# NVlabs/UMR

Hardware: NVIDIA H100
Metric: render fwd+bwd images/sec @256x256 1280-face mesh (higher is better)
Workload: dtype f32

## Files before the change

umr_b200/csrc/raster.cu:

```cuda
#include <cuda_runtime.h>
#include <stdint.h>

#include "common.cuh"
#include "umr_b200.h"

namespace umr {

constexpr int TILE = 16;
constexpr int CTA = TILE * TILE;
constexpr int CHUNK = 32;
constexpr int NSTAGE = 2;
constexpr int REC_F = 32;

constexpr int R_V = 0;
constexpr int R_INV = 9;
constexpr int R_SYM = 18;
constexpr int R_BOX = 24;
constexpr int R_FLG = 28;
constexpr int R_IZ2 = 29;

constexpr int NARROW_MAX_FACES = 65535;
template <typename IdxT>
__host__ __device__ constexpr int hdr_shift() { return sizeof(IdxT) == 2 ? 16 : 24; }
constexpr int FACE_WINDOW = 65536;
// ... 89 lines not shown
    if (valid) {
        float4* dst = reinterpret_cast<float4*>(rec + (size_t)i * REC_F);
#pragma unroll
        for (int k = 0; k < REC_F / 4; ++k)
            dst[k] = make_float4(out[4 * k], out[4 * k + 1], out[4 * k + 2], out[4 * k + 3]);
        box[i] = make_float4(xlo, xhi, ylo, yhi);
    }
    uint32_t k0 = ubox_key(xhi), k1 = ubox_key(-xlo), k2 = ubox_key(yhi), k3 = ubox_key(-ylo);
#pragma unroll
    for (int o = 16; o > 0; o >>= 1) {
        k0 = max(k0, __shfl_xor_sync(0xffffffffu, k0, o));
        k1 = max(k1, __shfl_xor_sync(0xffffffffu, k1, o));
        k2 = max(k2, __shfl_xor_sync(0xffffffffu, k2, o));
        k3 = max(k3, __shfl_xor_sync(0xffffffffu, k3, o));
    }
    if ((threadIdx.x & 31) == 0) {
        uint32_t* u = ubox + (size_t)blockIdx.y * 4;
        atomicMax(u + 0, k0); atomicMax(u + 1, k1); atomicMax(u + 2, k2); atomicMax(u + 3, k3);
    }
}

__device__ __forceinline__ bool tile_outside_union(const uint32_t* __restrict__ ubox, int b, const float* s_ext) {
    const uint4 u = __ldg(reinterpret_cast<const uint4*>(ubox) + b);
    if (u.x == 0xffffffffu || u.y == 0xffffffffu || u.z == 0xffffffffu || u.w == 0xffffffffu) return false;
    const float xhi = __uint_as_float(u.x), xlo = -__uint_as_float(u.y);
    const float yhi = __uint_as_float(u.z), ylo = -__uint_as_float(u.w);
    return s_ext[0] > xhi || s_ext[1] < xlo || s_ext[2] > yhi || s_ext[3] < ylo;
}

struct Frag {
    float w0, w1, w2;
    float t0, t1, t2;
    float sign, dx, dy, dis, D;
};

__device__ __forceinline__ float pixel_coord(int i, int S) {
    return __fdiv_rn((float)(2 * i + 1 - S), (float)S);
}

__device__ __forceinline__ bool fragment(const float* __restrict__ rc, float xp, float yp, float thr,
                                         float sigma, Frag& fr) {
    const float w0 = rc[R_INV + 0] * xp + rc[R_INV + 1] * yp + rc[R_INV + 2];
    const float w1 = rc[R_INV + 3] * xp + rc[R_INV + 4] * yp + rc[R_INV + 5];
    const float w2 = rc[R_INV + 6] * xp + rc[R_INV + 7] * yp + rc[R_INV + 8];
    fr.w0 = w0; fr.w1 = w1; fr.w2 = w2;
    const float fx0 = rc[0], fy0 = rc[1], fx1 = rc[3], fy1 = rc[4], fx2 = rc[6], fy2 = rc[7];
    const float s00 = rc[R_SYM + 0], s01 = rc[R_SYM + 1], s02 = rc[R_SYM + 2];
    const float s11 = rc[R_SYM + 3], s12 = rc[R_SYM + 4], s22 = rc[R_SYM + 5];
    float dx, dy, t0, t1, t2;
    if (w0 > 0 && w1 > 0 && w2 > 0 && w0 < 1 && w1 < 1 && w2 < 1) {
        float best = 100000000.f;
        {
            const float a0 = s00 - s01, a1 = s01 - s11, a2 = s02 - s12;
            float u0 = (w0 * a0 + w1 * a1 + w2 * a2 - a1) / (a0 - a1);
            float u1 = 1 - u0;
            float u2 = 0;
            u0 -= w0; u1 -= w1; u2 -= w2;
            const float ex = u0 * fx0 + u1 * fx1 + u2 * fx2;
            const float ey = u0 * fy0 + u1 * fy1 + u2 * fy2;
            const float d = ex * ex + ey * ey;
            dx = 0.f; dy = 0.f; t0 = t1 = t2 = 0.f;
            if (d < best) { best = d; dx = ex; dy = ey; t0 = u0; t1 = u1; t2 = u2; }
        }
        {
            const float a0 = s01 - s02, a1 = s11 - s12, a2 = s12 - s22;
            float u1 = (w0 * a0 + w1 * a1 + w2 * a2 - a2) / (a1 - a2);
            float u2 = 1 - u1;
            float u0 = 0;
            u0 -= w0; u1 -= w1; u2 -= w2;
            const float ex = u0 * fx0 + u1 * fx1 + u2 * fx2;
            const float ey = u0 * fy0 + u1 * fy1 + u2 * fy2;
            const float d = ex * ex + ey * ey;
            if (d < best) { best = d; dx = ex; dy = ey; t0 = u0; t1 = u1; t2 = u2; }
        }
        {
            const float a0 = s02 - s00, a1 = s12 - s01, a2 = s22 - s02;
            float u2 = (w0 * a0 + w1 * a1 + w2 * a2 - a0) / (a2 - a0);
            float u0 = 1 - u2;
            float u1 = 0;
            u0 -= w0; u1 -= w1; u2 -= w2;
            const float ex = u0 * fx0 + u1 * fx1 + u2 * fx2;
            const float ey = u0 * fy0 + u1 * fy1 + u2 * fy2;
            const float d = ex * ex + ey * ey;
            if (d < best) { best = d; dx = ex; dy = ey; t0 = u0; t1 = u1; t2 = u2; }
        }
        fr.sign = 1.f;
    } else {
        const uint32_t flg = __float_as_uint(rc[R_FLG]);
        int v0 = -1;
        if (w1 <= 0 && w2 <= 0) {
            v0 = 0;
            if ((flg & 1u) && (xp - fx0) * (fx2 - fx0) + (yp - fy0) * (fy2 - fy0) > 0) v0 = 2;
        } else if (w2 <= 0 && w0 <= 0) {
            v0 = 1;
            if ((flg & 2u) && (xp - fx1) * (fx0 - fx1) + (yp - fy1) * (fy0 - fy1) > 0) v0 = 0;
        } else if (w0 <= 0 && w1 <= 0) {
            v0 = 2;
            if ((flg & 4u) && (xp - fx2) * (fx1 - fx2) + (yp - fy2) * (fy1 - fy2) > 0) v0 = 1;
        } else if (w0 <= 0) v0 = 1;
        else if (w1 <= 0) v0 = 2;
        else if (w2 <= 0) v0 = 0;
        if (v0 < 0) v0 = w0 >= w1 ? (w0 >= w2 ? 0 : 2) : (w1 >= w2 ? 1 : 2);
        float u0, u1, u2;
        if (v0 == 0) {
            const float a0 = s00 - s01, a1 = s01 - s11, a2 = s02 - s12;
            u0 = (w0 * a0 + w1 * a1 + w2 * a2 - a1) / (a0 - a1);
            u1 = 1 - u0;
            u2 = 0;
        } else if (v0 == 1) {
            const float a0 = s01 - s02, a1 = s11 - s12, a2 = s12 - s22;
            u1 = (w0 * a0 + w1 * a1 + w2 * a2 - a2) / (a1 - a2);
            u2 = 1 - u1;
            u0 = 0;
        } else {
            const float a0 = s02 - s00, a1 = s12 - s01, a2 = s22 - s02;
            u2 = (w0 * a0 + w1 * a1 + w2 * a2 - a0) / (a2 - a0);
            u0 = 1 - u2;
            u1 = 0;
        }
        u0 = fminf(fmaxf(u0, 0.f), 1.f) - w0;
        u1 = fminf(fmaxf(u1, 0.f), 1.f) - w1;
        u2 = fminf(fmaxf(u2, 0.f), 1.f) - w2;
        t0 = u0; t1 = u1; t2 = u2;
        dx = t0 * fx0 + t1 * fx1 + t2 * fx2;
        dy = t0 * fy0 + t1 * fy1 + t2 * fy2;
        fr.sign = -1.f;
    }
    const float dis = dx * dx + dy * dy;
    if (fr.sign < 0 && dis >= thr) return false;
    fr.t0 = t0; fr.t1 = t1; fr.t2 = t2;
    fr.dx = dx; fr.dy = dy; fr.dis = dis;
    const float e = expf(-fr.sign * dis / sigma);
    fr.D = (float)(1. / (1. + (double)e));
    return true;
}


__device__ __forceinline__ void clip_bary(float& w0, float& w1, float& w2) {
    const float hi = (float)(1 - 1e-5), lo = (float)1e-5;
    w0 = fmaxf(fminf(w0, hi), lo);
    w1 = fmaxf(fminf(w1, hi), lo);
    w2 = fmaxf(fminf(w2, hi), lo);
    const float s = fmaxf(w0 + w1 + w2, lo);
    w0 /= s; w1 /= s; w2 /= s;
}

__device__ __forceinline__ float depth_of(const float* __restrict__ rc, float c0, float c1, float c2) {
    return __fdiv_rn(1.f, c0 / rc[2] + c1 / rc[5] + c2 / rc[8]);
}

__device__ __forceinline__ int texel_index(float c0, float c1, int R) {
    const int wx = (int)(c0 * R);
    const int wy = (int)(c1 * R);
    if ((c0 + c1) * R - wx - wy <= 1) return wy * R + wx;
    return (R - 1 - wy) * R + (R - 1 - wx);
}

struct Consts {
    float thr, sigma, gamma, near_, far_, inv_unused;
    float r_sigma, r_gamma, r_fn, r_nf;
    int F, T2, R, S, IS, aa, double_side;
    int dist, alpha, tex;
    int vec_store;
    size_t tex_bs;
    int tex_div;
};

constexpr int P2F_LIMBS = 4;
constexpr int P2F_LIMB_BITS = 26;
constexpr int P2F_FRAC_BITS = 96;
constexpr int P2F_DET_WORDS = 3 * P2F_LIMBS + 1;

__device__ __forceinline__ void red_add_u64(unsigned long long* addr, unsigned long long v) {
    asm volatile("red.global.add.u64 [%0], %1;" ::"l"(addr), "l"(v) : "memory");
}

__device__ __forceinline__ void red_fixed(unsigned long long* limbs, unsigned long long* bad, float v) {
// ... 1228 lines not shown
                        const float* aggrs_info, const float* grad_images, float* grad_faces, float* grad_textures,
                        const Consts& K, const PairBuf& pb) {
#define UMR_BWD2_GO(GEOMV, PREV) \
    k_raster_bwd2<RGBM, TG, TS, 3, GEOMV, PREV, IdxT><<<grid, BWD2_THREADS, 0, stream>>>(rec, textures, soft_colors, aggrs_info, grad_images, \
                                                                                    grad_faces, grad_textures, K, pb)
    if constexpr (TG && RGBM == 1) {
        if (pre) { if (grad_faces) UMR_BWD2_GO(true, true); else UMR_BWD2_GO(false, true); }
        else { if (grad_faces) UMR_BWD2_GO(true, false); else UMR_BWD2_GO(false, false); }
    } else if constexpr (TG) {
        if (grad_faces) UMR_BWD2_GO(true, false); else UMR_BWD2_GO(false, false);
    } else {
        UMR_BWD2_GO(true, false);
    }
#undef UMR_BWD2_GO
}

static int forward_impl(int tile_mode) { return tile_mode == 32 ? 4 : 3; }

extern "C" size_t umr_raster_workspace_bytes(int32_t B, int32_t F, int32_t image_size, int32_t anti_aliasing) {
    if (B <= 0 || F <= 0 || image_size <= 0) return 0;
    return ws_layout(B, F, image_size * (anti_aliasing ? 2 : 1)).total;
}

constexpr size_t PAIR_BLOCK_RESERVE = 1540;
extern "C" size_t umr_raster_pair_buffer_bytes(int32_t B, int32_t image_size, int32_t anti_aliasing,
                                               uint64_t capacity_blocks) {
    if (B <= 0 || image_size <= 0) return 0;
    const size_t blk = (size_t)BLK_F4 * sizeof(float4) + sizeof(uint32_t);
    return pair_layout(B, image_size * (anti_aliasing ? 2 : 1), (size_t)capacity_blocks).total +
           (size_t)capacity_blocks * (PAIR_BLOCK_RESERVE - blk) + 1024;
}

static int pair_texel_bits(const UmrRasterParams* p) {
    return (p->color_channels != 4 && forward_impl(p->tile_mode) == 4) ? 21 : 23;
}

static PairBuf make_pairbuf(const UmrRasterParams* p, int S) {
    PairBuf pb;
    pb.ctrl = nullptr; pb.tile_head = nullptr; pb.ulist = nullptr; pb.blk_hdr = nullptr; pb.recs = nullptr; pb.cap = 0;
    if (!p->pair_buffer || p->pair_buffer_bytes == 0 || ((uintptr_t)p->pair_buffer & 255) != 0) return pb;
    if (p->texture_size > (1 << pair_texel_bits(p))) return pb;
    size_t cap = pair_capacity(p->batch_size, S, (size_t)p->pair_buffer_bytes);
    if (cap > 0x7fff0000u) cap = 0x7fff0000u;
    if (cap < 4) return pb;
    const PairBufLayout L = pair_layout(p->batch_size, S, cap);
    char* base = (char*)p->pair_buffer;
    pb.ctrl = (uint32_t*)(base + L.ctrl_off);
    pb.tile_head = (int32_t*)(base + L.head_off);
    pb.ulist = (int32_t*)(base + L.ulist_off);
    pb.blk_hdr = (uint32_t*)(base + L.hdr_off);
    pb.recs = (float4*)(base + L.rec_off);
    pb.cap = (uint32_t)cap;
    return pb;
}

constexpr double TEXGRAD_PRE_RATIO_FULL = 160.0, TEXGRAD_PRE_RATIO_TEXONLY = 120.0;
static bool is_generic(const UmrRasterParams* p);
static int check_params(const UmrRasterParams* p) {
    if (!p) return UMR_ERR_BAD_ARG;
    if (p->batch_size <= 0 || p->num_faces <= 0 || p->texture_size <= 0 || p->image_size <= 0)
        return UMR_ERR_BAD_ARG;
    if (p->num_faces > UMR_RASTER_MAX_FACES || p->batch_size > 65535) return UMR_ERR_TOO_LARGE;
    if (p->func_id_dist < 0 || p->func_id_dist > 2 || p->func_id_alpha < 0 || p->func_id_alpha > 2 ||
        p->texture_sample_type < 0 || p->texture_sample_type > 1)
        return UMR_ERR_UNSUPPORTED;
    if (p->texture_sample_type == UMR_TEX_VERTEX && p->texture_size != 3) return UMR_ERR_BAD_ARG;
    if (p->shared_textures > 1 && p->batch_size % p->shared_textures != 0) return UMR_ERR_BAD_ARG;
// ... 441 lines not shown
```

umr_b200/csrc/raster_fwd3.cuh:

```cuda
#pragma once

namespace umr {

constexpr int FWD3_CTAS = 4;

template <int RGB, int NC = 3, typename IdxT = uint16_t, bool DET = false>
__global__ void __launch_bounds__(CTA, FWD3_CTAS) k_raster_fwd3(const float* __restrict__ rec_all, const float4* __restrict__ box_all,
                                                        const IdxT* __restrict__ clist, const int* __restrict__ ccount,
                                                        const float* __restrict__ textures, float* __restrict__ images,
                                                        float* __restrict__ colors_hi, float* __restrict__ aggrs,
                                                        float* __restrict__ p2f_acc, const uint32_t* __restrict__ ubox,
                                                        Consts K, float eps, float bg0, float bg1, float bg2, PairBuf pb,
                                                        int ncb, float bg3 = 0.f,
                                                        uint8_t* __restrict__ vis_mask = nullptr) {
    constexpr int NPL = NC + 1;
    constexpr bool VIS = RGB == 2;
    const float bgc[4] = {bg0, bg1, bg2, bg3};
    constexpr int WG = 16;
    __shared__ __align__(128) float s_wrec[NWARP * 2 * WG * REC_F];
    float* s_rec = s_wrec;
    __shared__ IdxT s_list[LCAP];
    __shared__ uint8_t s_meet[LCAP];
    __shared__ uint32_t s_boff[LCAP + 1];
    __shared__ float s_xp[TILE], s_yp[TILE], s_ext[4];
// ... 262 lines not shown
            for (int r = 0; mm; ++r) {
                const int e = __ffs(mm) - 1;
                mm &= mm - 1u;
                const int jl = base + e;
                const uint32_t meet = s_meet[jl];
                const float* rc = stage + r * REC_F;
                const float4 bb = *reinterpret_cast<const float4*>(rc + R_BOX);
                float a_x = 0.f, a_y = 0.f, a_w = 0.f;
                bool contrib = false, emit = false;
                Frag fr;
                float k0 = 0.f, k1 = 0.f, k2 = 0.f, zsave = 0.f;
                uint32_t tix = 0, front = 0;
                if (VIS) {
                    if (live && !(xp > bb.y || xp < bb.x || yp > bb.w || yp < bb.z)) {
                        const float w0 = rc[R_INV + 0] * xp + rc[R_INV + 1] * yp + rc[R_INV + 2];
                        const float w1 = rc[R_INV + 3] * xp + rc[R_INV + 4] * yp + rc[R_INV + 5];
                        const float w2 = rc[R_INV + 6] * xp + rc[R_INV + 7] * yp + rc[R_INV + 8];
                        const bool inside = w0 <= 1 && w0 >= 0 && w1 <= 1 && w1 >= 0 && w2 <= 1 && w2 >= 0;
                        if (inside && (K.double_side || (__float_as_uint(rc[R_FLG]) & 8u))) {
                            bool pass = w0 > 0 && w1 > 0 && w2 > 0 && w0 < 1 && w1 < 1 && w2 < 1;
                            if (!pass) pass = fragment(rc, xp, yp, K.thr, K.sigma, fr);
                            if (pass) {
                                k0 = w0; k1 = w1; k2 = w2;
                                clip_bary(k0, k1, k2);
                                const float zp = depth_of(rc, k0, k1, k2);
                                if (!(zp < K.near_ || zp > K.far_) && zp < zmin) {
                                    zmin = zp;
                                    fid = s_list[jl];
                                }
                            }
                        }
                    }
                } else if (live && !(xp > bb.y || xp < bb.x || yp > bb.w || yp < bb.z)) {
                    if (fragment(rc, xp, yp, K.thr, K.sigma, fr)) {
                        acc_a = (float)((double)acc_a * (1. - (double)fr.D));
                        k0 = fr.w0; k1 = fr.w1; k2 = fr.w2;
                        clip_bary(k0, k1, k2);
                        const float zp = depth_of(rc, k0, k1, k2);
                        if (!(zp < K.near_ || zp > K.far_)) {
                            emit = true;
                            front = (__float_as_uint(rc[R_FLG]) & 8u) ? 1u : 0u;
                            tix = (uint32_t)texel_index(k0, k1, K.R);
                            const int f = s_list[jl];
                            zsave = zp;
                            if (RGB == 0) {
                                const bool inside = fr.w0 <= 1 && fr.w0 >= 0 && fr.w1 <= 1 && fr.w1 >= 0 &&
                                                    fr.w2 <= 1 && fr.w2 >= 0;
                                if (zp < zmin && inside && (K.double_side || front)) {
                                    zmin = zp;
                                    fid = f;
                                    const float* tp = tex_img + ((size_t)f * K.T2 + tix) * NC;
#pragma unroll
                                    for (int k = 0; k < NC; ++k) col[k] = __ldg(tp + k);
                                }
                            } else {
                                const float zn = (K.far_ - zp) / (K.far_ - K.near_);
                                zsave = zn;
                                if (front || K.double_side) {
                                    float ed = 1.f;
                                    if (zn > smax) { ed = expf((smax - zn) / K.gamma); smax = zn; }
                                    const float ez = expf((zn - smax) / K.gamma);
                                    ssum = ed * ssum + ez * fr.D;
                                    const float a = ez * fr.D;
                                    if (a != 0.f || ed != 1.f) {
                                        a_x = a * gx; a_y = a * gy; a_w = a;
                                        contrib = a != 0.f;
                                        const float* tp = tex_img + ((size_t)f * K.T2 + tix) * NC;
#pragma unroll
                                        for (int k = 0; k < NC; ++k) col[k] = ed * col[k] + a * __ldg(tp + k);
                                    }
                                }
                            }
                        }
                    }
                }
                if (save) {
                    const uint32_t m = __ballot_sync(0xffffffffu, emit);
                    const uint32_t blk = segbase + s_boff[jl] + (uint32_t)__popc(meet & wlow);
                    if (emit) {
                        float4* dst = pb.recs + (size_t)blk * BLK_F4 + __popc(m & lt);
                        const float u0 = fr.t0 + fr.w0, u1 = fr.t1 + fr.w1, u2 = fr.t2 + fr.w2;
                        const uint32_t meta = (uint32_t)(lrow * TILE + lcol) | (tix << 8) | (front << 31);
                        dst[0] = make_float4(fr.D, fr.sign * fr.dx, fr.sign * fr.dy, zsave);
                        dst[32] = make_float4(u0, u1, u2, __uint_as_float(meta));
                    }
                    if (lane == 0) pb.blk_hdr[blk] = (uint32_t)s_list[jl] | ((uint32_t)__popc(m) << hdr_shift<IdxT>());
                }
                if (RGB == 1 && p2f_acc != nullptr) {
                    if (__any_sync(0xffffffffu, contrib)) {
                        a_x = warp_sum(a_x); a_y = warp_sum(a_y); a_w = warp_sum(a_w);
                        if (lane == r) { own_x += a_x; own_y += a_y; own_w += a_w; }
                    }
                }
            }
            if (RGB == 1 && p2f_acc != nullptr) {
                if (own_w != 0.f) {
                    const int e = __fns(m_cur, 0, lane + 1);
                    if constexpr (DET) {
                        red_p2f_fixed(reinterpret_cast<unsigned long long*>(p2f_acc) + ((size_t)b * F + s_list[base + e]) * P2F_DET_WORDS,
                                      own_x, own_y, own_w);
                    } else {
                    float* dst = p2f_acc + ((size_t)b * F + s_list[base + e]) * 4;
                    red_add4_global(dst, own_x, own_y, own_w, 0.f);
                    }
                }
            }
            __syncwarp();
            m_cur = m_next;
        }
        cp_async_wait<0>();
        __syncthreads();
    }
    if (tid == 0 && pb.cap > 0) pb.tile_head[tile_id] = head;

    const float alpha = (float)(1. - (double)acc_a);
    if (VIS) {
        if (vis_mask != nullptr && live) {
// ... 86 lines not shown
```

umr_b200/csrc/raster_fwd4.cuh:

```cuda
#pragma once

namespace umr {

constexpr int T4 = 32;
constexpr int FWD4_CAP = 1536;
constexpr int WG4 = 16;

__host__ __device__ inline size_t fwd4_dyn_smem(int F, size_t idx_bytes = 2) {
    return (size_t)(F < FWD4_CAP ? F : FWD4_CAP) * (8 + idx_bytes) + 16;
}

template <int RGB, typename IdxT = uint16_t>
__global__ void __launch_bounds__(CTA, 4) k_raster_fwd4(const float* __restrict__ rec_all, const float4* __restrict__ box_all,
                                                        const IdxT* __restrict__ clist, const int* __restrict__ ccount,
                                                        const float* __restrict__ textures, float* __restrict__ images,
                                                        float* __restrict__ colors_hi, float* __restrict__ aggrs,
                                                        float* __restrict__ p2f_acc, const uint32_t* __restrict__ ubox,
                                                        Consts K, float eps, float bg0, float bg1, float bg2, PairBuf pb,
                                                        int ncb) {
    extern __shared__ __align__(16) unsigned char smem_dyn[];
    const int F = K.F;
    const int LC = F < FWD4_CAP ? F : FWD4_CAP;
    uint32_t* s_boff = reinterpret_cast<uint32_t*>(smem_dyn);
    uint32_t* s_meet = s_boff + (LC + 1);
// ... 175 lines not shown
                const int base = g * WG4;
                m = __ballot_sync(0xffffffffu, lane < WG4 && base + lane < n && (s_meet[min(base + lane, n - 1)] & qbit));
                const int cntm = __popc(m);
                for (int r = lane >> 3; r < cntm; r += 4) {
                    const int e = __fns(m, 0, r + 1);
                    const int f = s_list[base + e];
                    cp_async16(wst + ((size_t)(g & 1) * WG4 + r) * REC_F + (lane & 7) * 4, rec_img + (size_t)f * REC_F + (lane & 7) * 4);
                }
            }
            cp_async_commit();
            return m;
        };
        uint32_t m_cur = issue(0);
        for (int g = 0; g < ngroup; ++g) {
            const uint32_t m_next = issue(g + 1);
            cp_async_wait<1>();
            __syncwarp();
            const int base = g * WG4;
            const float* stage = wst + (size_t)(g & 1) * WG4 * REC_F;
            float own_x = 0.f, own_y = 0.f, own_w = 0.f;
            uint32_t mm = m_cur;
            for (int r = 0; mm; ++r) {
                const int e = __ffs(mm) - 1;
                mm &= mm - 1u;
                const int jl = base + e;
                const float* rc = stage + r * REC_F;
                const float4 bb = *reinterpret_cast<const float4*>(rc + R_BOX);
                float a_x = 0.f, a_y = 0.f, a_w = 0.f;
                bool contrib = false, emit = false;
                Frag fr;
                float k0 = 0.f, k1 = 0.f, k2 = 0.f, zsave = 0.f;
                uint32_t tix = 0, front = 0;
                if (live && !(xp > bb.y || xp < bb.x || yp > bb.w || yp < bb.z)) {
                    if (fragment(rc, xp, yp, K.thr, K.sigma, fr)) {
                        acc_a = (float)((double)acc_a * (1. - (double)fr.D));
                        k0 = fr.w0; k1 = fr.w1; k2 = fr.w2;
                        clip_bary(k0, k1, k2);
                        const float zp = depth_of(rc, k0, k1, k2);
                        if (!(zp < K.near_ || zp > K.far_)) {
                            emit = true;
                            front = (__float_as_uint(rc[R_FLG]) & 8u) ? 1u : 0u;
                            tix = (uint32_t)texel_index(k0, k1, K.R);
                            const int f = s_list[jl];
                            zsave = zp;
                            if (RGB == 0) {
                                const bool inside = fr.w0 <= 1 && fr.w0 >= 0 && fr.w1 <= 1 && fr.w1 >= 0 &&
                                                    fr.w2 <= 1 && fr.w2 >= 0;
                                if (zp < zmin && inside && (K.double_side || front)) {
                                    zmin = zp;
                                    fid = f;
                                    const float* tp = tex_img + ((size_t)f * K.T2 + tix) * 3;
                                    c0 = __ldg(tp); c1 = __ldg(tp + 1); c2 = __ldg(tp + 2);
                                }
                            } else {
                                const float zn = (K.far_ - zp) / (K.far_ - K.near_);
                                zsave = zn;
                                if (front || K.double_side) {
                                    float ed = 1.f;
                                    if (zn > smax) { ed = expf((smax - zn) / K.gamma); smax = zn; }
                                    const float ez = expf((zn - smax) / K.gamma);
                                    ssum = ed * ssum + ez * fr.D;
                                    const float a = ez * fr.D;
                                    if (a != 0.f || ed != 1.f) {
                                        a_x = a * gx; a_y = a * gy; a_w = a;
                                        contrib = a != 0.f;
                                        const float* tp = tex_img + ((size_t)f * K.T2 + tix) * 3;
                                        c0 = ed * c0 + a * __ldg(tp);
                                        c1 = ed * c1 + a * __ldg(tp + 1);
                                        c2 = ed * c2 + a * __ldg(tp + 2);
                                    }
                                }
                            }
                        }
                    }
                }
                if (save) {
                    const uint32_t m = __ballot_sync(0xffffffffu, emit);
                    const uint32_t blk = segbase + s_boff[jl] + (uint32_t)__popc(s_meet[jl] & qlow);
                    if (emit) {
                        float4* dst = pb.recs + (size_t)blk * BLK_F4 + __popc(m & lt);
                        const float u0 = fr.t0 + fr.w0, u1 = fr.t1 + fr.w1, u2 = fr.t2 + fr.w2;
                        const uint32_t meta = (uint32_t)(lrow * T4 + lcol) | (tix << 10) | (front << 31);
                        dst[0] = make_float4(fr.D, fr.sign * fr.dx, fr.sign * fr.dy, zsave);
                        dst[32] = make_float4(u0, u1, u2, __uint_as_float(meta));
                    }
                    if (lane == 0) pb.blk_hdr[blk] = (uint32_t)s_list[jl] | ((uint32_t)__popc(m) << hdr_shift<IdxT>());
                }
                if (RGB == 1 && p2f_acc != nullptr) {
                    if (__any_sync(0xffffffffu, contrib)) {
                        a_x = warp_sum(a_x); a_y = warp_sum(a_y); a_w = warp_sum(a_w);
                        if (lane == r) { own_x += a_x; own_y += a_y; own_w += a_w; }
                    }
                }
            }
            if (RGB == 1 && p2f_acc != nullptr) {
                if (own_w != 0.f) {
                    const int e = __fns(m_cur, 0, lane + 1);
                    float* dst = p2f_acc + ((size_t)b * F + s_list[base + e]) * 4;
                    red_add_global(dst + 0, own_x);
                    red_add_global(dst + 1, own_y);
                    red_add_global(dst + 2, own_w);
                }
            }
            __syncwarp();
            m_cur = m_next;
        }
        cp_async_wait<0>();
        __syncwarp();
        st.acc_a = acc_a; st.ssum = ssum; st.smax = smax; st.c0 = c0; st.c1 = c1; st.c2 = c2; st.zmin = zmin; st.fid = fid;
    };

    auto store_block = [&](int q, const PixelState& st) {
        const int lcol = (q & 3) * 8 + (lane & 7), lrow = (q >> 2) * 4 + (lane >> 3);
        const int px = tx0 + lcol, py = ty0 + lrow;
        const bool live = px < S && py < S;
        const float alpha = (float)(1. - (double)st.acc_a);
        float o0, o1, o2, g0, g1;
// ... 136 lines not shown
```

umr_b200/csrc/raster_stream.cuh:

```cuda
#pragma once

namespace umr {

constexpr int CB = 64;
constexpr int LCAP = 512;
constexpr uint32_t SEG_NONE = 0xffffffffu;
constexpr int32_t TILE_EMPTY = -1, TILE_UNSAVED = -2;
constexpr int BLK_F4 = 64;

struct PairBuf {
    uint32_t* ctrl;
    int32_t* tile_head;
    int32_t* ulist;
    uint32_t* blk_hdr;
    float4* recs;
    uint32_t cap;
};

struct PairBufLayout {
    size_t ctrl_off, head_off, ulist_off, hdr_off, rec_off, total;
};
inline PairBufLayout pair_layout(int B, int S, size_t cap_blocks) {
    PairBufLayout L;
    const size_t nt = (size_t)((S + TILE - 1) / TILE) * ((S + TILE - 1) / TILE) * B;
    L.ctrl_off = 0;
    L.head_off = 256;
    L.ulist_off = L.head_off + align256(nt * sizeof(int32_t));
    L.hdr_off = L.ulist_off + align256(nt * sizeof(int32_t));
    L.rec_off = L.hdr_off + align256(cap_blocks * sizeof(uint32_t));
    L.total = L.rec_off + cap_blocks * (size_t)BLK_F4 * sizeof(float4);
    return L;
}
inline size_t pair_capacity(int B, int S, size_t bytes) {
    const PairBufLayout z = pair_layout(B, S, 0);
    if (bytes <= z.total + 512) return 0;
    size_t cap = (bytes - z.total - 512) / ((size_t)BLK_F4 * sizeof(float4) + sizeof(uint32_t));
    while (cap > 0 && pair_layout(B, S, cap).total > bytes) --cap;
    return cap;
}

template <typename IdxT>
// ... 142 lines not shown
        }
    };
    for (int i = warp; i < nc;) {
        scan_face(i);
        int nx = 0;
        if (lane == 0) nx = atomicAdd(&s_next, 1);
        i = __shfl_sync(0xffffffffu, nx, 0);
    }
    __syncthreads();
    bool bg = false;
    for (int i = tid; i < CB * CB; i += CTA) {
        const int row = i / CB, col = i - row * CB;
        if (row >= nrow || col >= ncol) continue;
        const unsigned long long key = s_z[i];
        if (key == ~0ull) { bg = true; continue; }
        uint8_t* m = vb + (uint32_t)(key & 0xffffffffull);
        if (*reinterpret_cast<volatile uint8_t*>(m) == 0) *m = 1;
    }
    if (bg) s_bg = 1;
    __syncthreads();
    if (tid == 0 && s_bg && *reinterpret_cast<volatile uint8_t*>(vb + F - 1) == 0) vb[F - 1] = 1;
}

template <int NC>
__device__ __forceinline__ void red_add_texel(float* gt, const float* v) {
    if (NC == 3) {
        red_add3_global(gt, v[0], v[1], v[2]);
    } else {
#pragma unroll
        for (int c = 0; c < NC; ++c) red_add_global(gt + c, v[c]);
    }
}

constexpr int BWD2_CTAS = 5;
constexpr int BWD2_THREADS = 256, BWD2_WARPS = BWD2_THREADS / 32;
template <int RGB, bool TEXGRAD, int TS, int NC = 3, bool GEOM = true, bool PRE = false, typename IdxT = uint16_t>
__global__ void __launch_bounds__(BWD2_THREADS, BWD2_CTAS) k_raster_bwd2(const float* __restrict__ rec_all, const float* __restrict__ textures,
                                                        const float* __restrict__ colors_hi,
                                                        const float* __restrict__ aggrs, const float* __restrict__ grad_images,
                                                        float* __restrict__ grad_faces, float* __restrict__ grad_tex, Consts K,
                                                        PairBuf pb) {
    constexpr int NPL = NC + 1, NV = 2 * NPL + 2;
    __shared__ float s_pix[NV][TS * TS];
    __shared__ float s_xp[TS], s_yp[TS];
    constexpr int NP = TS * TS;
    const int tid = threadIdx.x, lane = tid & 31, warp = tid >> 5;
    const int b = blockIdx.z;
    const int S = K.S, F = K.F;
    const size_t tile_id = ((size_t)b * gridDim.y + blockIdx.y) * gridDim.x + blockIdx.x;
    const int32_t head = __ldg(pb.tile_head + tile_id);
    if (head < 0) return;
    const int x0 = blockIdx.x * TS, y0 = blockIdx.y * TS;
    if (GEOM) {
        if (tid < TS) s_xp[tid] = pixel_coord(x0 + tid, S);
        else if (tid < 2 * TS) s_yp[tid - TS] = pixel_coord(S - 1 - (y0 + tid - TS), S);
    }
    for (int pi = tid; pi < NP; pi += BWD2_THREADS) {
        const int px = x0 + (pi % TS), py = y0 + (pi / TS);
        const size_t np = (size_t)S * S;
        float v[NV];
#pragma unroll
        for (int k = 0; k < NV; ++k) v[k] = (k == NV - 2) ? 1.f : 0.f;
        if (px < S && py < S) {
            const size_t p = (size_t)py * S + px;
            if (K.aa) {
                const size_t nq = (size_t)K.IS * K.IS;
                const size_t q = (size_t)(py >> 1) * K.IS + (px >> 1);
#pragma unroll
                for (int k = 0; k < NPL; ++k) v[k] = __ldg(grad_images + ((size_t)b * NPL + k) * nq + q) * 0.25f;
            } else {
#pragma unroll
                for (int k = 0; k < NPL; ++k) v[k] = __ldg(grad_images + ((size_t)b * NPL + k) * np + p);
            }
#pragma unroll
            for (int k = 0; k < NPL; ++k) v[NPL + k] = __ldg(colors_hi + ((size_t)b * NPL + k) * np + p);
            v[NV - 2] = __ldg(aggrs + ((size_t)b * 2 + 0) * np + p);
            v[NV - 1] = __ldg(aggrs + ((size_t)b * 2 + 1) * np + p);
        }
#pragma unroll
        for (int k = 0; k < NV; ++k) s_pix[k][pi] = v[k];
    }
    __syncthreads();
    const float* tex_img = textures + (size_t)(b / K.tex_div) * K.tex_bs;
    float* gtex_img = TEXGRAD ? grad_tex + (size_t)(b / K.tex_div) * K.tex_bs : nullptr;
    float* gf_img = grad_faces + (size_t)b * F * 9;
    const float* rec_img = GEOM ? rec_all + (size_t)b * F * REC_F : nullptr;
    auto prefetch_face = [&](int f) {
        if (lane >= 1 && lane < 4) asm volatile("prefetch.global.L1 [%0];" ::"l"(rec_img + (size_t)f * REC_F + 8 * lane));
    };

    float acc[9];
#pragma unroll
    for (int k = 0; k < 9; ++k) acc[k] = 0.f;
    int cur_f = -1;
    auto flush = [&]() {
        if (GEOM && cur_f >= 0) {
#pragma unroll
            for (int k = 0; k < 9; ++k) acc[k] = warp_sum(acc[k]);
            if (lane < 9) {
                float v = acc[0];
#pragma unroll
                for (int k = 1; k < 9; ++k) v = (lane == k) ? acc[k] : v;
                if (v != 0.f) red_add_global(gf_img + (size_t)cur_f * 9 + lane, v);
            }
#pragma unroll
            for (int k = 0; k < 9; ++k) acc[k] = 0.f;
        }
    };

    uint32_t seg = (uint32_t)head;
    while (seg != SEG_NONE) {
        const uint32_t NB = __ldg(pb.blk_hdr + seg), next = __ldg(pb.blk_hdr + seg + 1);
        const uint32_t per = (NB + BWD2_WARPS - 1) / BWD2_WARPS;
        const uint32_t kbeg = min(NB, warp * per), kend = min(NB, kbeg + per);
        const uint32_t* hdrs = pb.blk_hdr + seg + 2;
        uint32_t k = kbeg, kwin = kbeg;
        uint32_t hw = (kbeg + lane < kend) ? __ldg(hdrs + kbeg + lane) : 0u;
        int o = 0;
        auto plan = [&](int& f_out, bool& act_out, const float4*& src_out) -> bool {
            while (k < kend) {
                if (k >= kwin + 32u) {
// ... 8 lines not shown
                constexpr uint32_t HM = (1u << HS) - 1u;
                const int a0 = (int)(h0 >> HS) - o;
                if (a0 <= 0) { ++k; o = 0; continue; }
                const int f = (int)(h0 & HM);
                int a1 = 0, a2 = 0, a3 = 0, nchain = 1;
                if (k + 1 < wend && ((h1 >> HS) == 0 || (int)(h1 & HM) == f)) {
                    a1 = (int)(h1 >> HS); nchain = 2;
                    if (k + 2 < wend && ((h2 >> HS) == 0 || (int)(h2 & HM) == f)) {
                        a2 = (int)(h2 >> HS); nchain = 3;
                        if (k + 3 < wend && ((h3 >> HS) == 0 || (int)(h3 & HM) == f)) { a3 = (int)(h3 >> HS); nchain = 4; }
                    }
                }
                const int p1 = a0, p2 = a0 + a1, p3 = p2 + a2, p4 = p3 + a3;
                int bi, pos;
                if (lane < p1) { bi = 0; pos = lane + o; }
                else if (lane < p2) { bi = 1; pos = lane - p1; }
                else if (lane < p3) { bi = 2; pos = lane - p2; }
                else { bi = 3; pos = lane - p3; }
                f_out = f;
                act_out = lane < p4;
                src_out = pb.recs + (size_t)(seg + 2 + k + bi) * BLK_F4 + pos;
                int left = min(32, p4), i = 0;
                const int av[4] = {a0, a1, a2, a3};
#pragma unroll
                for (int q = 0; q < 4; ++q) {
                    if (i == q && q < nchain && left >= av[q]) { left -= av[q]; ++i; }
                }
                k += (uint32_t)i;
                o = (i == 0) ? o + left : ((i < nchain) ? left : 0);
                return true;
            }
            return false;
        };
        auto prefetch2 = [&](bool act, const float4* p) {
            if (act) {
                asm volatile("prefetch.global.L1 [%0];" ::"l"(p));
                asm volatile("prefetch.global.L1 [%0];" ::"l"(p + 32));
            }
        };
        int f_c = 0, f_n = 0;
        bool act_c = false, act_n = false;
        const float4 *src_c = nullptr, *src_n = nullptr;
        bool have = plan(f_c, act_c, src_c);
        if (have) prefetch2(act_c, src_c);
        if (GEOM && have) prefetch_face(f_c);
        while (have) {
            const bool have_n = plan(f_n, act_n, src_n);
            if (have_n) prefetch2(act_n, src_n);
            const int f = f_c;
            if (f != cur_f) { flush(); cur_f = f; }
            if (GEOM && have_n && f_n != f) prefetch_face(f_n);
            int pre_tix = -1;
            float pre_v[NC];
#pragma unroll
            for (int c = 0; c < NC; ++c) pre_v[c] = 0.f;
            if (act_c) {
                const float4* src = src_c;
                const float4 r0 = __ldg(src), r1 = __ldg(src + 32);
                const float D = r0.x, sdx = r0.y, sdy = r0.z, zn = r0.w;
                const uint32_t meta = __float_as_uint(r1.w);
                const int pix = TS == 16 ? (int)(meta & 0xffu) : (int)(meta & 0x3ffu);
                const int tix = TS == 16 ? (int)((meta >> 8) & 0x7fffffu) : (int)((meta >> 10) & 0x1fffffu);
                const bool front = (meta >> 31) != 0u;
                const float* sp = &s_pix[0][pix];
                float Cxy = 0.f;
                if (GEOM) {
                    const float g3 = sp[NC * NP];
                    const float one_m_a = 1 - sp[(2 * NC + 1) * NP];
                    Cxy = (one_m_a == 0.f || g3 == 0.f) ? g3 * one_m_a : g3 * __fdividef(one_m_a, fmaxf(1 - D, 1e-6f));
                }
                if (RGB == 0) {
                    if ((float)f == sp[(NV - 1) * NP]) {
                        if (TEXGRAD) {
                            float* gt = gtex_img + ((size_t)f * K.T2 + tix) * NC;
                            float g_[NC];
#pragma unroll
                            for (int c = 0; c < NC; ++c) g_[c] = sp[c * NP];
                            red_add_texel<NC>(gt, g_);
                        }
                    }
                } else if (front || K.double_side) {
                    float g[NC];
                    bool any = false;
#pragma unroll
                    for (int c = 0; c < NC; ++c) { g[c] = sp[c * NP]; any = any || g[c] != 0.f; }
                    if (any) {
                        const float s = __fdividef(D * expf((zn - sp[(NV - 1) * NP]) * K.r_gamma), sp[(NV - 2) * NP]);
                        if (s != 0.f) {
                            const size_t to = ((size_t)f * K.T2 + tix) * NC;
                            if (TEXGRAD) {
                                if (PRE) {
                                    pre_tix = tix;
#pragma unroll
                                    for (int c = 0; c < NC; ++c) pre_v[c] = s * g[c];
                                } else {
                                    float sg[NC];
#pragma unroll
                                    for (int c = 0; c < NC; ++c) sg[c] = s * g[c];
                                    red_add_texel<NC>(gtex_img + to, sg);
                                }
                            }
                            float Crgb = 0.f;
                            if (GEOM) {
#pragma unroll
                                for (int c = 0; c < NC; ++c) Crgb += g[c] * (__ldg(tex_img + to + c) - sp[(NPL + c) * NP]);
                                Crgb *= s;
                            }
                            if (GEOM && Crgb != 0.f) {
                                Cxy += __fdividef(Crgb, D);
                                const float zp = K.far_ - zn * (K.far_ - K.near_);
                                const float Cz = Crgb * K.r_gamma * K.r_nf * zp * zp;
                                const float* q = rec_img + (size_t)f * REC_F;
                                const float xp = s_xp[pix % TS], yp = s_yp[pix / TS];
                                float k0 = __ldg(q + R_INV + 0) * xp + __ldg(q + R_INV + 1) * yp + __ldg(q + R_INV + 2);
                                float k1 = __ldg(q + R_INV + 3) * xp + __ldg(q + R_INV + 4) * yp + __ldg(q + R_INV + 5);
                                float k2 = __ldg(q + R_INV + 6) * xp + __ldg(q + R_INV + 7) * yp + __ldg(q + R_INV + 8);
                                clip_bary(k0, k1, k2);
                                acc[2] += Cz * (k0 * __ldg(q + R_IZ2 + 0));
                                acc[5] += Cz * (k1 * __ldg(q + R_IZ2 + 1));
                                acc[8] += Cz * (k2 * __ldg(q + R_IZ2 + 2));
                            }
                        }
                    }
                }
                if (GEOM) {
                    Cxy *= D * (1 - D) * K.r_sigma;
                    const float q = 2 * Cxy;
                    acc[0] += q * r1.x * sdx;
                    acc[1] += q * r1.x * sdy;
                    acc[3] += q * r1.y * sdx;
                    acc[4] += q * r1.y * sdy;
                    acc[6] += q * r1.z * sdx;
                    acc[7] += q * r1.z * sdy;
                }
            }
            if (PRE && TEXGRAD && RGB == 1) {
                const bool has = pre_tix >= 0;
                if (__any_sync(0xffffffffu, has)) {
                    const uint32_t lt_ = (1u << lane) - 1u;
                    const uint32_t pm = __match_any_sync(0xffffffffu, has ? (uint32_t)pre_tix : (0x80000000u | (uint32_t)lane));
                    const bool leader = (pm & lt_) == 0u;
                    uint32_t rest = (has && leader) ? (pm & ~(1u << lane)) : 0u;
                    float sum[NC];
#pragma unroll
                    for (int c = 0; c < NC; ++c) sum[c] = pre_v[c];
                    while (__any_sync(0xffffffffu, rest != 0u)) {
                        const int src = rest ? __ffs(rest) - 1 : lane;
                        const bool take = rest != 0u;
                        rest &= rest - 1u;
#pragma unroll
                        for (int c = 0; c < NC; ++c) {
                            const float t = __shfl_sync(0xffffffffu, pre_v[c], src);
                            if (take) sum[c] += t;
                        }
                    }
                    if (has && leader) {
                        float* gt = gtex_img + ((size_t)f * K.T2 + pre_tix) * NC;
                        red_add_texel<NC>(gt, sum);
                    }
                }
            }
            f_c = f_n; act_c = act_n; src_c = src_n; have = have_n;
        }
        seg = next;
    }
    flush();
// ... 4 lines not shown
```

umr_b200/raster.py:

```python
import ctypes
import math
import os

import torch

from . import _lib

FUNC_DIST = {"hard": 0, "barycentric": 1, "euclidean": 2}
FUNC_RGB = {"hard": 0, "softmax": 1}
FUNC_ALPHA = {"hard": 0, "sum": 1, "prod": 2}
FUNC_SAMPLE = {"surface": 0, "vertex": 1}


_profile_sink = None


class _EventPair(object):

    __slots__ = ("start", "stop")

    def __init__(self):
        lib = _lib.load()
        self.start, self.stop = ctypes.c_void_p(), ctypes.c_void_p()
        _lib.check(lib.umr_event_create(ctypes.byref(self.start)), "umr_event_create")
# ... 36 lines not shown
    out = {"fwd": [], "bwd": []}
    for kind, ev in sink or []:
        out[kind].append(ev.elapsed_ms())
    if sink is not None:
        del sink[:]
    return out


PAIR_CAND_PER_PIXEL = float(os.environ.get("UMR_PAIR_CAND_PER_PIXEL", "8.0"))
FORWARD_TILE = int(os.environ.get("UMR_FORWARD_TILE", "0"))
_PAIR_MAX_GB = os.environ.get("UMR_PAIR_MAX_GB")
_pair_max = {}


def pair_max_bytes(device=None):
    if _PAIR_MAX_GB is not None:
        return int(float(_PAIR_MAX_GB) * (1 << 30))
    dev = torch.device("cuda" if device is None else device)
    idx = dev.index if dev.index is not None else torch.cuda.current_device()
    if idx not in _pair_max:
        _pair_max[idx] = torch.cuda.get_device_properties(idx).total_memory // 4
    return _pair_max[idx]


def pair_buffer_bytes(B, image_size, anti_aliasing, cand_per_pixel=None, blocks_per_image=None, device=None):
    lib = _lib.load()
    S = int(image_size) * (2 if anti_aliasing else 1)
    cpp = PAIR_CAND_PER_PIXEL if cand_per_pixel is None else cand_per_pixel
    tiles = B * ((S + 15) // 16) ** 2
    if blocks_per_image is not None:
        blocks = int(B * blocks_per_image * PAIR_HEADROOM) + 2 * tiles + 64
    else:
        blocks = int(B * S * S * cpp / 32.0) + 2 * tiles + 64
    nbytes = lib.umr_raster_pair_buffer_bytes(B, int(image_size), 1 if anti_aliasing else 0, blocks)
    return min(int(nbytes), pair_max_bytes(device))


PAIR_HEADROOM = float(os.environ.get("UMR_PAIR_HEADROOM", "1.35"))
PAIR_ADAPTIVE = os.environ.get("UMR_PAIR_ADAPTIVE", "1") != "0"
_pair_need = {}
_pair_pending = []


def _pair_poll():
    keep = []
    for key, B, host, ev in _pair_pending:
        if ev.query():
            need = float(host[0]) / max(B, 1)
            _pair_need[key] = max(_pair_need.get(key, 0.0), need)
        else:
            keep.append((key, B, host, ev))
    _pair_pending[:] = keep


def _pair_record(key, B, pairs):
    if not PAIR_ADAPTIVE or torch.cuda.is_current_stream_capturing() or len(_pair_pending) > 64:
        return
    host = torch.empty(2, dtype=torch.int32, pin_memory=True)
    host.copy_(pairs[:8].view(torch.int32), non_blocking=True)
    ev = torch.cuda.Event()
    ev.record()
    _pair_pending.append((key, B, host, ev))


def _stream_ptr(device):
    return ctypes.c_void_p(torch.cuda.current_stream(device).cuda_stream)

# ... 161 lines not shown
```

Before: 20980.

## Compress per-pair records to one float4 and recompute edge terms in backward

The forward pass now stores only D, depth, the edge parameter q and a meta word holding a 2-bit edge id, one float4 per pair instead of two. The backward kernel recomputes barycentrics, closest-edge offsets and signed distance from face data that each warp stages in shared memory when the face changes. This halves pair-buffer traffic and footprint, and the buffer sizing is halved to match. In exchange it adds recompute work, shrinks the texel-index bits by two, and lowers the backward occupancy hint from 5 to 4 CTAs.

```diff
diff --git a/umr_b200/csrc/raster.cu b/umr_b200/csrc/raster.cu
--- a/umr_b200/csrc/raster.cu
+++ b/umr_b200/csrc/raster.cu
@@ -145,12 +145,15 @@
     float w0, w1, w2;
     float t0, t1, t2;
     float sign, dx, dy, dis, D;
+    float q;
+    uint32_t e;
 };
 
 __device__ __forceinline__ float pixel_coord(int i, int S) {
     return __fdiv_rn((float)(2 * i + 1 - S), (float)S);
 }
 
+template <bool EDGE = false>
 __device__ __forceinline__ bool fragment(const float* __restrict__ rc, float xp, float yp, float thr,
                                          float sigma, Frag& fr) {
     const float w0 = rc[R_INV + 0] * xp + rc[R_INV + 1] * yp + rc[R_INV + 2];
@@ -160,12 +163,15 @@
     const float fx0 = rc[0], fy0 = rc[1], fx1 = rc[3], fy1 = rc[4], fx2 = rc[6], fy2 = rc[7];
     const float s00 = rc[R_SYM + 0], s01 = rc[R_SYM + 1], s02 = rc[R_SYM + 2];
     const float s11 = rc[R_SYM + 3], s12 = rc[R_SYM + 4], s22 = rc[R_SYM + 5];
-    float dx, dy, t0, t1, t2;
+    float dx, dy, t0, t1, t2, q;
+    uint32_t edge;
     if (w0 > 0 && w1 > 0 && w2 > 0 && w0 < 1 && w1 < 1 && w2 < 1) {
         float best = 100000000.f;
         {
             const float a0 = s00 - s01, a1 = s01 - s11, a2 = s02 - s12;
             float u0 = (w0 * a0 + w1 * a1 + w2 * a2 - a1) / (a0 - a1);
+            float qk;
+            if constexpr (EDGE) qk = u0;
             float u1 = 1 - u0;
             float u2 = 0;
             u0 -= w0; u1 -= w1; u2 -= w2;
@@ -173,29 +179,43 @@
             const float ey = u0 * fy0 + u1 * fy1 + u2 * fy2;
             const float d = ex * ex + ey * ey;
             dx = 0.f; dy = 0.f; t0 = t1 = t2 = 0.f;
-            if (d < best) { best = d; dx = ex; dy = ey; t0 = u0; t1 = u1; t2 = u2; }
+            if constexpr (EDGE) { q = 0.f; edge = 3u; }
+            if (d < best) {
+                best = d; dx = ex; dy = ey; t0 = u0; t1 = u1; t2 = u2;
+                if constexpr (EDGE) { q = qk; edge = 0u; }
+            }
         }
         {
             const float a0 = s01 - s02, a1 = s11 - s12, a2 = s12 - s22;
             float u1 = (w0 * a0 + w1 * a1 + w2 * a2 - a2) / (a1 - a2);
+            float qk;
+            if constexpr (EDGE) qk = u1;
             float u2 = 1 - u1;
             float u0 = 0;
             u0 -= w0; u1 -= w1; u2 -= w2;
             const float ex = u0 * fx0 + u1 * fx1 + u2 * fx2;
             const float ey = u0 * fy0 + u1 * fy1 + u2 * fy2;
             const float d = ex * ex + ey * ey;
-            if (d < best) { best = d; dx = ex; dy = ey; t0 = u0; t1 = u1; t2 = u2; }
+            if (d < best) {
+                best = d; dx = ex; dy = ey; t0 = u0; t1 = u1; t2 = u2;
+                if constexpr (EDGE) { q = qk; edge = 1u; }
+            }
         }
         {
             const float a0 = s02 - s00, a1 = s12 - s01, a2 = s22 - s02;
             float u2 = (w0 * a0 + w1 * a1 + w2 * a2 - a0) / (a2 - a0);
+            float qk;
+            if constexpr (EDGE) qk = u2;
             float u0 = 1 - u2;
             float u1 = 0;
             u0 -= w0; u1 -= w1; u2 -= w2;
             const float ex = u0 * fx0 + u1 * fx1 + u2 * fx2;
             const float ey = u0 * fy0 + u1 * fy1 + u2 * fy2;
             const float d = ex * ex + ey * ey;
-            if (d < best) { best = d; dx = ex; dy = ey; t0 = u0; t1 = u1; t2 = u2; }
+            if (d < best) {
+                best = d; dx = ex; dy = ey; t0 = u0; t1 = u1; t2 = u2;
+                if constexpr (EDGE) { q = qk; edge = 2u; }
+            }
         }
         fr.sign = 1.f;
     } else {
@@ -220,17 +240,21 @@
             u0 = (w0 * a0 + w1 * a1 + w2 * a2 - a1) / (a0 - a1);
             u1 = 1 - u0;
             u2 = 0;
+            if constexpr (EDGE) q = u0;
         } else if (v0 == 1) {
             const float a0 = s01 - s02, a1 = s11 - s12, a2 = s12 - s22;
             u1 = (w0 * a0 + w1 * a1 + w2 * a2 - a2) / (a1 - a2);
             u2 = 1 - u1;
             u0 = 0;
+            if constexpr (EDGE) q = u1;
         } else {
             const float a0 = s02 - s00, a1 = s12 - s01, a2 = s22 - s02;
             u2 = (w0 * a0 + w1 * a1 + w2 * a2 - a0) / (a2 - a0);
             u0 = 1 - u2;
             u1 = 0;
-        }
+            if constexpr (EDGE) q = u2;
+        }
+        if constexpr (EDGE) edge = (uint32_t)v0;
         u0 = fminf(fmaxf(u0, 0.f), 1.f) - w0;
         u1 = fminf(fmaxf(u1, 0.f), 1.f) - w1;
         u2 = fminf(fmaxf(u2, 0.f), 1.f) - w2;
@@ -243,6 +267,7 @@
     if (fr.sign < 0 && dis >= thr) return false;
     fr.t0 = t0; fr.t1 = t1; fr.t2 = t2;
     fr.dx = dx; fr.dy = dy; fr.dis = dis;
+    if constexpr (EDGE) { fr.q = q; fr.e = edge; }
     const float e = expf(-fr.sign * dis / sigma);
     fr.D = (float)(1. / (1. + (double)e));
     return true;
@@ -256,6 +281,28 @@
     w2 = fmaxf(fminf(w2, hi), lo);
     const float s = fmaxf(w0 + w1 + w2, lo);
     w0 /= s; w1 /= s; w2 /= s;
+}
+
+__device__ __forceinline__ void edge_terms(float fx0, float fy0, float fx1, float fy1, float fx2, float fy2, float w0,
+                                           float w1, float w2, float q, uint32_t e, float& t0, float& t1, float& t2,
+                                           float& sdx, float& sdy) {
+    const bool inside = w0 > 0 && w1 > 0 && w2 > 0 && w0 < 1 && w1 < 1 && w2 < 1;
+    const float qb = 1 - q;
+    float c0 = e == 0u ? q : (e == 1u ? 0.f : qb);
+    float c1 = e == 0u ? qb : (e == 1u ? q : 0.f);
+    float c2 = e == 0u ? 0.f : (e == 1u ? qb : q);
+    if (!inside) {
+        c0 = fminf(fmaxf(c0, 0.f), 1.f);
+        c1 = fminf(fmaxf(c1, 0.f), 1.f);
+        c2 = fminf(fmaxf(c2, 0.f), 1.f);
+    }
+    t0 = c0 - w0; t1 = c1 - w1; t2 = c2 - w2;
+    float dx = t0 * fx0 + t1 * fx1 + t2 * fx2;
+    float dy = t0 * fy0 + t1 * fy1 + t2 * fy2;
+    if (e == 3u) { t0 = t1 = t2 = 0.f; dx = 0.f; dy = 0.f; }
+    const float sign = inside ? 1.f : -1.f;
+    sdx = sign * dx;
+    sdy = sign * dy;
 }
 
 __device__ __forceinline__ float depth_of(const float* __restrict__ rc, float c0, float c1, float c2) {
@@ -1550,7 +1597,7 @@
 }
 
 static int pair_texel_bits(const UmrRasterParams* p) {
-    return (p->color_channels != 4 && forward_impl(p->tile_mode) == 4) ? 21 : 23;
+    return (p->color_channels != 4 && forward_impl(p->tile_mode) == 4) ? 19 : 21;
 }
 
 static PairBuf make_pairbuf(const UmrRasterParams* p, int S) {
diff --git a/umr_b200/csrc/raster_fwd3.cuh b/umr_b200/csrc/raster_fwd3.cuh
--- a/umr_b200/csrc/raster_fwd3.cuh
+++ b/umr_b200/csrc/raster_fwd3.cuh
@@ -318,7 +318,7 @@
                         }
                     }
                 } else if (live && !(xp > bb.y || xp < bb.x || yp > bb.w || yp < bb.z)) {
-                    if (fragment(rc, xp, yp, K.thr, K.sigma, fr)) {
+                    if (fragment<true>(rc, xp, yp, K.thr, K.sigma, fr)) {
                         acc_a = (float)((double)acc_a * (1. - (double)fr.D));
                         k0 = fr.w0; k1 = fr.w1; k2 = fr.w2;
                         clip_bary(k0, k1, k2);
@@ -365,10 +365,8 @@
                     const uint32_t blk = segbase + s_boff[jl] + (uint32_t)__popc(meet & wlow);
                     if (emit) {
                         float4* dst = pb.recs + (size_t)blk * BLK_F4 + __popc(m & lt);
-                        const float u0 = fr.t0 + fr.w0, u1 = fr.t1 + fr.w1, u2 = fr.t2 + fr.w2;
-                        const uint32_t meta = (uint32_t)(lrow * TILE + lcol) | (tix << 8) | (front << 31);
-                        dst[0] = make_float4(fr.D, fr.sign * fr.dx, fr.sign * fr.dy, zsave);
-                        dst[32] = make_float4(u0, u1, u2, __uint_as_float(meta));
+                        const uint32_t meta = (uint32_t)(lrow * TILE + lcol) | (tix << 8) | (fr.e << 29) | (front << 31);
+                        *dst = make_float4(fr.D, zsave, fr.q, __uint_as_float(meta));
                     }
                     if (lane == 0) pb.blk_hdr[blk] = (uint32_t)s_list[jl] | ((uint32_t)__popc(m) << hdr_shift<IdxT>());
                 }
diff --git a/umr_b200/csrc/raster_fwd4.cuh b/umr_b200/csrc/raster_fwd4.cuh
--- a/umr_b200/csrc/raster_fwd4.cuh
+++ b/umr_b200/csrc/raster_fwd4.cuh
@@ -231,7 +231,7 @@
                 float k0 = 0.f, k1 = 0.f, k2 = 0.f, zsave = 0.f;
                 uint32_t tix = 0, front = 0;
                 if (live && !(xp > bb.y || xp < bb.x || yp > bb.w || yp < bb.z)) {
-                    if (fragment(rc, xp, yp, K.thr, K.sigma, fr)) {
+                    if (fragment<true>(rc, xp, yp, K.thr, K.sigma, fr)) {
                         acc_a = (float)((double)acc_a * (1. - (double)fr.D));
                         k0 = fr.w0; k1 = fr.w1; k2 = fr.w2;
                         clip_bary(k0, k1, k2);
@@ -278,10 +278,8 @@
                     const uint32_t blk = segbase + s_boff[jl] + (uint32_t)__popc(s_meet[jl] & qlow);
                     if (emit) {
                         float4* dst = pb.recs + (size_t)blk * BLK_F4 + __popc(m & lt);
-                        const float u0 = fr.t0 + fr.w0, u1 = fr.t1 + fr.w1, u2 = fr.t2 + fr.w2;
-                        const uint32_t meta = (uint32_t)(lrow * T4 + lcol) | (tix << 10) | (front << 31);
-                        dst[0] = make_float4(fr.D, fr.sign * fr.dx, fr.sign * fr.dy, zsave);
-                        dst[32] = make_float4(u0, u1, u2, __uint_as_float(meta));
+                        const uint32_t meta = (uint32_t)(lrow * T4 + lcol) | (tix << 10) | (fr.e << 29) | (front << 31);
+                        *dst = make_float4(fr.D, zsave, fr.q, __uint_as_float(meta));
                     }
                     if (lane == 0) pb.blk_hdr[blk] = (uint32_t)s_list[jl] | ((uint32_t)__popc(m) << hdr_shift<IdxT>());
                 }
diff --git a/umr_b200/csrc/raster_stream.cuh b/umr_b200/csrc/raster_stream.cuh
--- a/umr_b200/csrc/raster_stream.cuh
+++ b/umr_b200/csrc/raster_stream.cuh
@@ -6,7 +6,7 @@
 constexpr int LCAP = 512;
 constexpr uint32_t SEG_NONE = 0xffffffffu;
 constexpr int32_t TILE_EMPTY = -1, TILE_UNSAVED = -2;
-constexpr int BLK_F4 = 64;
+constexpr int BLK_F4 = 32;
 
 struct PairBuf {
     uint32_t* ctrl;
@@ -215,7 +215,7 @@
     }
 }
 
-constexpr int BWD2_CTAS = 5;
+constexpr int BWD2_CTAS = 4;
 constexpr int BWD2_THREADS = 256, BWD2_WARPS = BWD2_THREADS / 32;
 template <int RGB, bool TEXGRAD, int TS, int NC = 3, bool GEOM = true, bool PRE = false, typename IdxT = uint16_t>
 __global__ void __launch_bounds__(BWD2_THREADS, BWD2_CTAS) k_raster_bwd2(const float* __restrict__ rec_all, const float* __restrict__ textures,
@@ -226,6 +226,7 @@
     constexpr int NPL = NC + 1, NV = 2 * NPL + 2;
     __shared__ float s_pix[NV][TS * TS];
     __shared__ float s_xp[TS], s_yp[TS];
+    __shared__ float s_face[BWD2_WARPS][REC_F];
     constexpr int NP = TS * TS;
     const int tid = threadIdx.x, lane = tid & 31, warp = tid >> 5;
     const int b = blockIdx.z;
@@ -269,7 +270,7 @@
     float* gf_img = grad_faces + (size_t)b * F * 9;
     const float* rec_img = GEOM ? rec_all + (size_t)b * F * REC_F : nullptr;
     auto prefetch_face = [&](int f) {
-        if (lane >= 1 && lane < 4) asm volatile("prefetch.global.L1 [%0];" ::"l"(rec_img + (size_t)f * REC_F + 8 * lane));
+        if (lane < 4) asm volatile("prefetch.global.L1 [%0];" ::"l"(rec_img + (size_t)f * REC_F + 8 * lane));
     };
 
     float acc[9];
@@ -344,37 +345,48 @@
             }
             return false;
         };
-        auto prefetch2 = [&](bool act, const float4* p) {
-            if (act) {
-                asm volatile("prefetch.global.L1 [%0];" ::"l"(p));
-                asm volatile("prefetch.global.L1 [%0];" ::"l"(p + 32));
-            }
+        auto prefetch_rec = [&](bool act, const float4* p) {
+            if (act) asm volatile("prefetch.global.L1 [%0];" ::"l"(p));
         };
         int f_c = 0, f_n = 0;
         bool act_c = false, act_n = false;
         const float4 *src_c = nullptr, *src_n = nullptr;
         bool have = plan(f_c, act_c, src_c);
-        if (have) prefetch2(act_c, src_c);
+        if (have) prefetch_rec(act_c, src_c);
         if (GEOM && have) prefetch_face(f_c);
         while (have) {
             const bool have_n = plan(f_n, act_n, src_n);
-            if (have_n) prefetch2(act_n, src_n);
+            if (have_n) prefetch_rec(act_n, src_n);
             const int f = f_c;
-            if (f != cur_f) { flush(); cur_f = f; }
+            if (f != cur_f) {
+                flush();
+                cur_f = f;
+                if (GEOM) {
+                    __syncwarp();
+                    s_face[warp][lane] = __ldg(rec_img + (size_t)f * REC_F + lane);
+                    __syncwarp();
+                }
+            }
             if (GEOM && have_n && f_n != f) prefetch_face(f_n);
             int pre_tix = -1;
             float pre_v[NC];
 #pragma unroll
             for (int c = 0; c < NC; ++c) pre_v[c] = 0.f;
             if (act_c) {
-                const float4* src = src_c;
-                const float4 r0 = __ldg(src), r1 = __ldg(src + 32);
-                const float D = r0.x, sdx = r0.y, sdy = r0.z, zn = r0.w;
-                const uint32_t meta = __float_as_uint(r1.w);
+                const float4 r0 = __ldg(src_c);
+                const float D = r0.x, zn = r0.y;
+                const uint32_t meta = __float_as_uint(r0.w);
                 const int pix = TS == 16 ? (int)(meta & 0xffu) : (int)(meta & 0x3ffu);
-                const int tix = TS == 16 ? (int)((meta >> 8) & 0x7fffffu) : (int)((meta >> 10) & 0x1fffffu);
+                const int tix = TS == 16 ? (int)((meta >> 8) & 0x1fffffu) : (int)((meta >> 10) & 0x7ffffu);
                 const bool front = (meta >> 31) != 0u;
                 const float* sp = &s_pix[0][pix];
+                const float* fq = s_face[warp];
+                auto bary = [&](float& w0, float& w1, float& w2) {
+                    const float xp = s_xp[pix % TS], yp = s_yp[pix / TS];
+                    w0 = fq[R_INV + 0] * xp + fq[R_INV + 1] * yp + fq[R_INV + 2];
+                    w1 = fq[R_INV + 3] * xp + fq[R_INV + 4] * yp + fq[R_INV + 5];
+                    w2 = fq[R_INV + 6] * xp + fq[R_INV + 7] * yp + fq[R_INV + 8];
+                };
                 float Cxy = 0.f;
                 if (GEOM) {
                     const float g3 = sp[NC * NP];
@@ -422,28 +434,31 @@
                                 Cxy += __fdividef(Crgb, D);
                                 const float zp = K.far_ - zn * (K.far_ - K.near_);
                                 const float Cz = Crgb * K.r_gamma * K.r_nf * zp * zp;
-                                const float* q = rec_img + (size_t)f * REC_F;
-                                const float xp = s_xp[pix % TS], yp = s_yp[pix / TS];
-                                float k0 = __ldg(q + R_INV + 0) * xp + __ldg(q + R_INV + 1) * yp + __ldg(q + R_INV + 2);
-                                float k1 = __ldg(q + R_INV + 3) * xp + __ldg(q + R_INV + 4) * yp + __ldg(q + R_INV + 5);
-                                float k2 = __ldg(q + R_INV + 6) * xp + __ldg(q + R_INV + 7) * yp + __ldg(q + R_INV + 8);
+                                float k0, k1, k2;
+                                bary(k0, k1, k2);
                                 clip_bary(k0, k1, k2);
-                                acc[2] += Cz * (k0 * __ldg(q + R_IZ2 + 0));
-                                acc[5] += Cz * (k1 * __ldg(q + R_IZ2 + 1));
-                                acc[8] += Cz * (k2 * __ldg(q + R_IZ2 + 2));
+                                acc[2] += Cz * (k0 * fq[R_IZ2 + 0]);
+                                acc[5] += Cz * (k1 * fq[R_IZ2 + 1]);
+                                acc[8] += Cz * (k2 * fq[R_IZ2 + 2]);
                             }
                         }
                     }
                 }
                 if (GEOM) {
+                    float w0, w1, w2, t0, t1, t2, sdx, sdy;
+                    bary(w0, w1, w2);
+                    edge_terms(fq[R_V + 0], fq[R_V + 1], fq[R_V + 3], fq[R_V + 4],
+                               fq[R_V + 6], fq[R_V + 7], w0, w1, w2, r0.z, (meta >> 29) & 3u, t0, t1, t2,
+                               sdx, sdy);
+                    const float u0 = t0 + w0, u1 = t1 + w1, u2 = t2 + w2;
                     Cxy *= D * (1 - D) * K.r_sigma;
                     const float q = 2 * Cxy;
-                    acc[0] += q * r1.x * sdx;
-                    acc[1] += q * r1.x * sdy;
-                    acc[3] += q * r1.y * sdx;
-                    acc[4] += q * r1.y * sdy;
-                    acc[6] += q * r1.z * sdx;
-                    acc[7] += q * r1.z * sdy;
+                    acc[0] += q * u0 * sdx;
+                    acc[1] += q * u0 * sdy;
+                    acc[3] += q * u1 * sdx;
+                    acc[4] += q * u1 * sdy;
+                    acc[6] += q * u2 * sdx;
+                    acc[7] += q * u2 * sdy;
                 }
             }
             if (PRE && TEXGRAD && RGB == 1) {
diff --git a/umr_b200/raster.py b/umr_b200/raster.py
--- a/umr_b200/raster.py
+++ b/umr_b200/raster.py
@@ -92,7 +92,7 @@
         blocks = int(B * blocks_per_image * PAIR_HEADROOM) + 2 * tiles + 64
     else:
         blocks = int(B * S * S * cpp / 32.0) + 2 * tiles + 64
-    nbytes = lib.umr_raster_pair_buffer_bytes(B, int(image_size), 1 if anti_aliasing else 0, blocks)
+    nbytes = lib.umr_raster_pair_buffer_bytes(B, int(image_size), 1 if anti_aliasing else 0, (blocks + 1) // 2)
     return min(int(nbytes), pair_max_bytes(device))
 
 
```

Result: faster. 21820 (median of 6 runs) (+4.0%).
